# als244/ResNet

Measured on AMD Instinct MI355X. Metric: images/sec ResNet-50 fp32 224x224 batch256, higher is better.
Workload: dtype f32

## Files before the change

include/resnet_mi.h:

```cpp
#ifndef RESNET_MI_H
#define RESNET_MI_H
#include <stddef.h>
#include <stdint.h>

#ifdef __cplusplus
extern "C" {
#endif

typedef struct {
    char **labels;
    char **synsets;
    int *counts;
    int n_classes;
} Class_Metadata;

typedef struct {
    int input;
    int init_kernel_dim;
    int init_conv_filters;
    int init_conv_stride;
    int init_maxpool_dim;
    int init_maxpool_stride;
    int n_conv_blocks;
    int *is_block_spatial_reduction;
// ... 208 lines not shown
int mi_op_bn_fwd_add_relu(const float *x, const float *gamma, const float *beta, const float *residual, float *means,
                          float *vars, float *y, int N, int C, int H, float eps);
int mi_op_bn_bwd(const float *x, const float *gamma, const float *beta, const float *means, const float *vars,
                 const float *dy, const float *mask_src, float *dx, float *dgamma, float *dbeta, int N, int C, int H,
                 float eps, int mask_mode);
int mi_op_bn_bwd_gate(const float *x, const float *gamma, const float *beta, const float *means, const float *vars,
                      const float *dy, const float *mask_src, float *gated_out, float *dx, float *dgamma, float *dbeta, int N,
                      int C, int H, float eps);
int mi_op_maxpool_fwd(const float *x, float *y, int *max_inds, int N, int C, int H, int k, int stride);
int mi_op_maxpool_bwd(const int *max_inds, const float *dy, float *dx, int N, int C, int H, int k, int stride);
int mi_op_avgpool_fwd(const float *x, float *y, int N, int C, int H);
int mi_op_avgpool_bwd(const float *dy, float *dx, int N, int C, int H);
int mi_op_relu_deriv(const float *x, const float *up, float *out, size_t n);
int mi_op_matmul(const float *A, const float *B, float *out, int m, int k, int n);
int mi_op_matmul_lt(const float *A_kxm, const float *B, float *out, int m, int k, int n);
int mi_op_matmul_rt(const float *A, const float *B_nxk, float *out, int m, int k, int n);
int mi_op_softmax(const float *x, float *out, int N, int L);
int mi_op_ce_deriv(const float *pred, const int *labels, float *d, int N, int L);
int mi_op_adam(float *p, const float *g, float *m, float *v, size_t n, float lr, float wd, float b1, float b2,
               float cur_b1, float cur_b2, float eps, int *nan_flag_dev);
int mi_op_nhwc_to_nchw(const float *in, float *out, int N, int H, int W, int C);
int mi_debug_lds_fill(uint32_t word);
int mi_debug_poison_lds(void);
int mi_debug_lds_probe(uint32_t word, size_t out[4]);
int mi_debug_lds_geometry(size_t out[3]);
int mi_debug_lds_fill_mode(int on, uint32_t word);
size_t mi_debug_lds_fills(void);
int mi_debug_redzone(size_t zone_bytes, int fill_byte);
int mi_debug_redzone_check(void);
void mi_debug_redzone_stats(size_t *allocs_checked, size_t *zone_bytes_checked, size_t *live);
int mi_debug_trace_names(char *buf, size_t cap);
void mi_debug_trace_clear(void);
int mi_debug_conv_plan(int op, int N, int C, int H, int K, int k, int stride, int out[9]);
int mi_op_fill_uniform(float *out, size_t n, uint64_t seed, float lo, float hi);
enum { MI_ROUTE_DEFAULT = 0, MI_ROUTE_CL = 1, MI_ROUTE_CL2 = 2, MI_ROUTE_PW = 3 };
int mi_conv_plan(int dtype, int route, int op, int N, int C, int H, int K, int k, int stride, int out[7]);
enum { MI_FWD_F32, MI_FWD_BF16, MI_FWD_CL, MI_FWD_STEM_F32, MI_FWD_STEM_BF16, MI_FWD_PW  };
enum { MI_DG_F32, MI_DG_BF16, MI_DG_CL, MI_DG_CL2 };
enum { MI_WG_F32, MI_WG_BF16, MI_WG_CL, MI_WG_CL2, MI_WG_STEM_F32, MI_WG_STEM_BF16 };
int mi_layer_routes(int dtype, int policy, int N, int C, int H, int K, int k, int stride, int site, int out[4]);
enum {
    MI_K_NONE,
    MI_K_IGEMM,
    MI_K_GEMM1X1,
    MI_K_DCONV,
    MI_K_WGRADC,
    MI_K_WGRAD,
    MI_K_BGEMM,
    MI_K_PW_WGRAD,
    MI_K_CL_CONV,
    MI_K_CL_DGRAD2,
    MI_K_CL_WGRAD,
    MI_K_CL_WGRAD2,
    MI_K_ST32_FWD,
    MI_K_ST32_WGRAD,
    MI_K_ST_FWD,
    MI_K_ST_WGRAD
};
int mi_layer_kernels(int dtype, int policy, int N, int C, int H, int K, int k, int stride, int site, int out[3]);


enum { MI_DTYPE_F32 = 0, MI_DTYPE_BF16 = 1 };
int mi_trainer_set_dtype(Train_ResNet *t, int dtype);
int mi_trainer_get_dtype(const Train_ResNet *t);
enum { MI_STORE_FAST = 0, MI_STORE_RECOMPUTE_BN = 1, MI_STORE_FULL = 2 };
int mi_trainer_set_store_policy(Train_ResNet *t, int policy);
// ... 173 lines not shown
```

resnet_amd/binding.py:

```python
import ctypes as C
import os

_HERE = os.path.dirname(os.path.abspath(__file__))
LIB_PATH = os.environ.get("RESNET_MI_LIB") or os.path.join(_HERE, "libresnet_mi.so")

_fp = C.POINTER(C.c_float)
_ip = C.POINTER(C.c_int)


class Dims(C.Structure):
    _fields_ = [("input", C.c_int), ("init_kernel_dim", C.c_int), ("init_conv_filters", C.c_int),
                ("init_conv_stride", C.c_int), ("init_maxpool_dim", C.c_int), ("init_maxpool_stride", C.c_int),
                ("n_conv_blocks", C.c_int), ("is_block_spatial_reduction", _ip), ("final_depth", C.c_int),
                ("output", C.c_int)]


class BatchNorm(C.Structure):
    _fields_ = [("spatial_dim", C.c_int), ("depth", C.c_int), ("gamma", _fp), ("beta", _fp)]


class ConvBlock(C.Structure):
    _fields_ = [("incoming_filters", C.c_int), ("incoming_spatial_dim", C.c_int), ("reduced_depth", C.c_int),
                ("expanded_depth", C.c_int), ("stride", C.c_int), ("depth_reduction", _fp),
                ("norm_depth_reduction", C.POINTER(BatchNorm)), ("spatial", _fp), ("norm_spatial", C.POINTER(BatchNorm)),
# ... 191 lines not shown
    "mi_free": (None, [_vp]),
    "mi_op_conv_fwd": (_i, [_vp, _vp, _vp, _i, _i, _i, _i, _i, _i]),
    "mi_op_conv_dgrad": (_i, [_vp, _vp, _vp, _i, _i, _i, _i, _i, _i, _i]),
    "mi_op_conv_wgrad": (_i, [_vp, _vp, _vp, _i, _i, _i, _i, _i, _i]),
    "mi_op_bn_fwd": (_i, [_vp, _vp, _vp, _vp, _vp, _vp, _i, _i, _i, _f, _i]),
    "mi_op_bn_fwd_add_relu": (_i, [_vp, _vp, _vp, _vp, _vp, _vp, _vp, _i, _i, _i, _f]),
    "mi_op_bn_bwd": (_i, [_vp] * 10 + [_i, _i, _i, _f, _i]),
    "mi_op_bn_bwd_gate": (_i, [_vp] * 11 + [_i, _i, _i, _f]),
    "mi_op_maxpool_fwd": (_i, [_vp, _vp, _vp, _i, _i, _i, _i, _i]),
    "mi_op_maxpool_bwd": (_i, [_vp, _vp, _vp, _i, _i, _i, _i, _i]),
    "mi_op_avgpool_fwd": (_i, [_vp, _vp, _i, _i, _i]),
    "mi_op_avgpool_bwd": (_i, [_vp, _vp, _i, _i, _i]),
    "mi_op_relu_deriv": (_i, [_vp, _vp, _vp, _sz]),
    "mi_op_matmul": (_i, [_vp, _vp, _vp, _i, _i, _i]),
    "mi_op_matmul_lt": (_i, [_vp, _vp, _vp, _i, _i, _i]),
    "mi_op_matmul_rt": (_i, [_vp, _vp, _vp, _i, _i, _i]),
    "mi_op_softmax": (_i, [_vp, _vp, _i, _i]),
    "mi_op_ce_deriv": (_i, [_vp, _vp, _vp, _i, _i]),
    "mi_op_adam": (_i, [_vp, _vp, _vp, _vp, _sz, _f, _f, _f, _f, _f, _f, _f, _vp]),
    "mi_op_nhwc_to_nchw": (_i, [_vp, _vp, _i, _i, _i, _i]),
    "mi_op_fill_uniform": (_i, [_vp, _sz, _u64, _f, _f]),
    "mi_debug_poison_lds": (_i, []),
    "mi_debug_lds_fill": (_i, [C.c_uint32]),
    "mi_debug_lds_probe": (_i, [C.c_uint32, C.POINTER(_sz)]),
    "mi_debug_lds_geometry": (_i, [C.POINTER(_sz)]),
    "mi_debug_lds_fill_mode": (_i, [_i, C.c_uint32]),
    "mi_debug_lds_fills": (_sz, []),
    "mi_debug_redzone": (_i, [_sz, _i]),
    "mi_debug_redzone_check": (_i, []),
    "mi_debug_redzone_stats": (None, [C.POINTER(_sz)] * 3),
    "mi_debug_trace_names": (_i, [C.c_char_p, _sz]),
    "mi_debug_trace_clear": (None, []),
    "mi_debug_conv_plan": (_i, [_i] * 7 + [_vp]),
    "mi_conv_plan": (_i, [_i] * 9 + [_vp]),
    "mi_layer_routes": (_i, [_i] * 9 + [_vp]),
    "mi_layer_kernels": (_i, [_i] * 9 + [_vp]),
    "mi_debug_trainer_routes": (_i, [_T, _vp, _i]),
    "mi_trainer_set_dtype": (_i, [_T, _i]),
    "mi_trainer_get_dtype": (_i, [_T]),
    "mi_trainer_set_store_policy": (_i, [_T, _i]),
    "mi_trainer_activation_bytes": (_sz, [_T]),
    "mi_trainer_device_bytes": (_sz, [_T]),
    "mi_clear_error": (None, []),
    "mi_trainer_check_errors": (_i, [_T]),
    "mi_trainer_end_epoch": (None, [_T, _f, _f, _f]),
    "mi_trainer_set_optimizer": (_i, [_T, _i, _f, _f]),
    "mi_trainer_get_optimizer": (_i, [_T]),
    "mi_op_loss_head": (_i, [_vp, _vp, _vp, _vp, _vp, _vp, _i, _i, _f, _i, _vp, _vp]),
    "mi_trainer_set_loss": (_i, [_T, _f, _i, _i]),
    "mi_trainer_metrics": (_i, [_T, C.POINTER(MiLossMetrics), C.POINTER(MiLossMetrics), _i]),
    "mi_trainer_track_running_stats": (_i, [_T, _i, _f]),
    "mi_bn_unbias": (_f, [C.c_int64]),
    "mi_op_bn_running_update": (_i, [_vp, _vp, _vp, _vp, _i, _vp, _i, _f]),
    "mi_trainer_running_stats_channels": (_i, [_T]),
    "mi_trainer_get_running_stats": (_i, [_T, _vp, _vp]),
    "mi_trainer_set_running_stats": (_i, [_T, _vp, _vp]),
    "mi_trainer_running_updates": (C.c_int64, [_T]),
    "mi_trainer_eval_forward": (_i, [_T, _vp, _vp, _i, _i]),
    "mi_trainer_eval_metrics": (_i, [_T, C.POINTER(MiLossMetrics), C.POINTER(MiLossMetrics), _i]),
    "mi_trainer_eval_u8": (_i, [_T, _vp, _vp, C.c_int64, _i, _i, C.POINTER(MiLossMetrics)]),
    "mi_ema_weight": (_f, [C.c_double, _i, C.c_int64]),
    "mi_op_ema_update": (_i, [_vp, _vp, _sz, _f]),
    "mi_op_exchange": (_i, [_vp, _vp, _sz]),
    "mi_debug_ema_geometry": (None, [C.POINTER(_sz)]),
    "mi_trainer_set_ema": (_i, [_T, C.c_double, _i, _i]),
    "mi_trainer_ema_reset": (_i, [_T]),
# ... 108 lines not shown
```

resnet_amd/csrc/kernels_igemm.hip:

```cpp
#include "mi_common.hpp"
#include <type_traits>
#include "mi_device.h"

typedef float f32x16 __attribute__((ext_vector_type(16)));
typedef float pf4 __attribute__((ext_vector_type(4)));

enum { IG_FWD = 0, IG_DGRAD = 1, IG_WGRAD = 2 };

struct IgArgs {
    int N, C, K, H, W, Ho, Wo;
    int HW, P;
    int ncols;
    int mtiles;
    int tiles;
    int ctiles;
    int klen;
    FastDiv fdP, fdWo, fdM;
    int full, tsplit, tklen, cpt;
    FastDiv fdTs, fdCpt;
    float *tailbuf;
    float *bn_part;
    int bn_np;
    const float *bnb_x, *bnb_mask, *bnb_mean;
    float *bnb_part;
    int bnb_np;
};

__device__ __forceinline__ float ig_half_sum32(float v) {
    v += __int_as_float(__builtin_amdgcn_update_dpp(0, __float_as_int(v), 0xB1, 0xF, 0xF, true));
    v += __int_as_float(__builtin_amdgcn_update_dpp(0, __float_as_int(v), 0x4E, 0xF, 0xF, true));
    v += __int_as_float(__builtin_amdgcn_update_dpp(0, __float_as_int(v), 0x141, 0xF, 0xF, true));
    v += __int_as_float(__builtin_amdgcn_update_dpp(0, __float_as_int(v), 0x140, 0xF, 0xF, true));
    v += __int_as_float(__builtin_amdgcn_update_dpp(0, __float_as_int(v), 0x142, 0xA, 0xF, true));
    return v;
}

__device__ __forceinline__ void ig_half_stats(float x, int nv, int l31, float &mean, float &m2) {
    const float s = __shfl(x, (int)(threadIdx.x & 32), 64);
    const float d = l31 < nv ? x - s : 0.f;
    float sd = d, sq = d * d;
#pragma unroll
    for (int o = 16; o > 0; o >>= 1) { sd += __shfl_xor(sd, o, 64); sq += __shfl_xor(sq, o, 64); }
    const float inv = nv > 0 ? 1.0f / (float)nv : 0.f;
    mean = s + sd * inv;
    m2 = fmaxf(sq - sd * sd * inv, 0.f);
    if (nv <= 0) { mean = 0.f; m2 = 0.f; }
}
__device__ __forceinline__ void ig_merge(float &na, float &ma, float &qa, float nb, float mb, float qb) {
    const float n = na + nb;
    if (n > 0.f) {
        const float dlt = mb - ma, f = nb / n;
        ma = ma + dlt * f;
        qa = qa + qb + dlt * dlt * na * f;
    }
    na = n;
}

#define IG_BK 32
#ifdef IG_STAMP
__device__ unsigned long long ig_stamps[8 * 16384];
#define IG_T(slot) do { if (threadIdx.x == 0 && blockIdx.x < 16384 && blockIdx.y == 0) ig_stamps[blockIdx.x * 8 + (slot)] = __builtin_amdgcn_s_memtime(); } while (0)
#else
#define IG_T(slot) do { } while (0)
#endif
#ifndef IG_ABLATE
#define IG_ABLATE 0
#endif

template <int MODE, int KS, int S, int WMW, bool VBP = false>
__global__ void __launch_bounds__(256)
igemm_kernel(const float *__restrict__ Aop, const float *__restrict__ Bop, float *__restrict__ Out,
             const float *__restrict__ addend, const IgArgs g) {
    constexpr int BM = 64 * WMW;
    constexpr int TN = WMW == 2 ? 2 : 1;
    constexpr int WNC = 32 * TN;
    constexpr int T = KS * KS, PAD = KS / 2;
    constexpr int LDA = (MODE == IG_WGRAD) ? BM + 1 : BM + 4;
    constexpr int LDB = (MODE == IG_WGRAD) ? 129 : 132;
    constexpr int NA4 = BM / 32;
    constexpr int NAS = BM / 8;
    constexpr bool VB = VBP && KS == 1 && MODE != IG_WGRAD;
    constexpr bool CT64 = VBP && MODE == IG_WGRAD;
    extern __shared__ __attribute__((aligned(16))) float ig_smem[];
    float *As = ig_smem;
    float *Bs = ig_smem + 2 * IG_BK * LDA;
    const int tid = threadIdx.x, lane = tid & 63;
    const int wave = __builtin_amdgcn_readfirstlane(tid >> 6);
    const int wm = WMW == 2 ? wave >> 1 : 0, wn = WMW == 2 ? wave & 1 : wave;

    IG_T(0);
    uint32_t L = blockIdx.x;
    int tail_id = -1, it0 = 0, nt_slice = 0;
    uint32_t wg_split = blockIdx.y;
    if (MODE != IG_WGRAD && g.tsplit > 1 && L >= (uint32_t)g.full) {
        tail_id = (int)(L - (uint32_t)g.full);
        const uint32_t tl = fd_div((uint32_t)tail_id, g.fdTs);
        const int z = tail_id - (int)tl * g.tsplit;
        L = (uint32_t)g.full + tl;
        it0 = z * g.tklen;
        nt_slice = g.tklen;
    } else if (MODE == IG_WGRAD && gridDim.y >= 8) {
        const uint32_t T_ = gridDim.x, tot = T_ * gridDim.y, per = tot >> 3;
// ... 251 lines not shown
            __builtin_amdgcn_sched_barrier(0);
            if (grp < 8) { if (st) stash_part(buf ^ 1, grp); }
            else { if (ft) fetch_part(grp - 8); }
#pragma unroll
            for (int i = 0; i < 2; i++)
#pragma unroll
                for (int j = 0; j < TN; j++)
                    acc[i][j] = __builtin_amdgcn_mfma_f32_32x32x2f32(av[cur][i], bv[cur][j], acc[i][j], 0, 0, 0);
            __builtin_amdgcn_sched_barrier(0);
        }
        __syncthreads();
    };
    {
        constexpr std::true_type Y{};
        constexpr std::false_type NO{};
        int it = 0;
        for (; it + 2 < ntiles; it++) kstep(Y, Y, it & 1);
        if (it + 1 < ntiles) { kstep(Y, NO, it & 1); it++; }
        if (it < ntiles) kstep(NO, NO, it & 1);
    }

    IG_T(2);
    if (MODE != IG_WGRAD && tail_id >= 0) {
        float *tb = g.tailbuf + (size_t)tail_id * (BM * 128);
#pragma unroll
        for (int j = 0; j < TN; j++)
#pragma unroll
            for (int i = 0; i < 2; i++)
#pragma unroll
                for (int r = 0; r < 16; r++)
                    tb[(wm * 64 + i * 32 + (r & 3) + 8 * (r >> 2) + 4 * (lane >> 5)) * 128 + wn * WNC + j * 32 + (lane & 31)] = acc[i][j][r];
        return;
    }
    if (MODE == IG_DGRAD && S == 1 && g.bnb_part) {
        constexpr int PPT = 4 / WMW;
        if ((g.P & 3) == 0) {
            constexpr int CPR = WNC / 4, RPI = 64 / CPR, PITCH = WNC + 4;
            float *img = ig_smem + wave * (32 * PITCH);
            const int c4 = (lane % CPR) * 4, r0 = lane / CPR;
            const int col = n0 + wn * WNC + c4;
            const bool cok = col < g.ncols;
            const uint32_t jc = cok ? (uint32_t)col : 0u;
            const uint32_t nimg = fd_div(jc, g.fdP);
            const size_t coff = (size_t)nimg * g.C * g.HW + (jc - nimg * g.P);
            const size_t pplane = (size_t)g.bnb_np * g.C;
#pragma unroll
            for (int i = 0; i < 2; i++) {
#pragma unroll
                for (int j = 0; j < TN; j++)
#pragma unroll
                    for (int r = 0; r < 16; r++)
                        img[((r & 3) + 8 * (r >> 2) + 4 * (lane >> 5)) * PITCH + j * 32 + (lane & 31)] = acc[i][j][r];
#pragma unroll
                for (int ps = 0; ps < 32 / RPI; ps++) {
                    const int rl = ps * RPI + r0;
                    const int row = m0 + wm * 64 + i * 32 + rl;
                    const size_t o = coff + (size_t)row * g.HW;
                    const pf4 z = {0.f, 0.f, 0.f, 0.f};
                    pf4 v = *(const pf4 *)(img + rl * PITCH + c4);
                    pf4 xv = z, mv = z;
                    if (cok) {
                        if (addend) v += *(const pf4 *)(addend + o);
                        xv = *(const pf4 *)(g.bnb_x + o);
                        mv = *(const pf4 *)(g.bnb_mask + o);
                    }
                    const float mean = g.bnb_mean[row];
                    float s1 = 0.f, s2 = 0.f;
// ... 184 lines not shown
        for (int i = 0; i < 8; i++) {
            const size_t o = coff + (size_t)(m0 + row0 + i) * rstride;
            float r = v[i];
            if (MODE == IG_DGRAD && addend) r += addend[o];
            Out[o] = r;
        }
    }
    if (MODE == IG_FWD && g.bn_part) {
        constexpr int PPT = BM == 128 ? 2 : 4;
        const int lane = threadIdx.x & 63, l31 = lane & 31;
        const int c32 = (int)ct * 128 + (int)(threadIdx.x & 127 & ~31);
        const int nv = min(32, max(0, g.ncols - c32));
        const size_t plane = (size_t)g.bn_np * g.K;
#pragma unroll
        for (int i = 0; i < 8; i++) {
            float mj, qj, nj = (float)nv;
            ig_half_stats(v[i], nv, l31, mj, qj);
            int pp = (int)(threadIdx.x & 127) >> 5;
            if (PPT == 2) {
                const float n2 = __shfl_xor(nj, 32, 64), m2o = __shfl_xor(mj, 32, 64), q2 = __shfl_xor(qj, 32, 64);
                if (lane == 0) ig_merge(nj, mj, qj, n2, m2o, q2);
                pp >>= 1;
            }
            if (PPT == 2 ? lane == 0 : l31 == 0) {
                const size_t o = (size_t)(ct * PPT + pp) * g.K + m0 + row0 + i;
                g.bn_part[o] = nj;
                g.bn_part[plane + o] = mj;
                g.bn_part[2 * plane + o] = qj;
            }
        }
    }
}

template <int T>
__global__ void __launch_bounds__(256)
igemm_wt_kernel(const float *__restrict__ w, float *__restrict__ out, int K, int C, int to_tck) {
    __shared__ float tile[32][T * 32 + 1];
    const int k0 = blockIdx.y * 32, c0 = blockIdx.x * 32;
    for (int e = threadIdx.x; e < 32 * T * 32; e += 256) {
        const int kr = e / (T * 32), x = e - kr * (T * 32);
        tile[kr][x] = w[((size_t)(k0 + kr) * C + c0) * T + x];
    }
    __syncthreads();
    for (int e = threadIdx.x; e < T * 32 * 32; e += 256) {
        const int t = e >> 10, u = (e >> 5) & 31, v = e & 31;
        if (to_tck) out[((size_t)t * C + c0 + u) * K + k0 + v] = tile[v][u * T + t];
        else out[((size_t)t * K + k0 + u) * C + c0 + v] = tile[u][v * T + t];
    }
}

__global__ void __launch_bounds__(256)
igemm_wt_all_kernel(const mid_wt_entry *__restrict__ entries, const int *__restrict__ tile_entry) {
    __shared__ float tile[32][9 * 32 + 1];
    const mid_wt_entry E = entries[tile_entry[blockIdx.x]];
    const int tl = (int)blockIdx.x - E.tile0, ctiles = E.C / 32, T = E.T;
    const int c0 = (tl % ctiles) * 32, k0 = (tl / ctiles) * 32, row = T * 32;
    for (int e = threadIdx.x; e < 32 * row; e += 256) {
        const int kr = e / row, x = e - kr * row;
        tile[kr][x] = E.w[((size_t)(k0 + kr) * E.C + c0) * T + x];
    }
    __syncthreads();
    for (int e = threadIdx.x; e < T * 1024; e += 256) {
        const int t = e >> 10, u = (e >> 5) & 31, v = e & 31;
        if (E.fwd) E.fwd[((size_t)t * E.C + c0 + u) * E.K + k0 + v] = tile[v][u * T + t];
        if (E.dgrad) E.dgrad[((size_t)t * E.K + k0 + u) * E.C + c0 + v] = tile[u][v * T + t];
    }
// ... 195 lines not shown
    const int bm = (op == IGOP_FWD || stride == 1) ? igemm_pick_bm(M, mi_cdiv(g.ncols, 128), k * k * (red / IG_BK), k) : (M % 128 == 0 ? 128 : 64);
    g.mtiles = M / bm;
    g.tiles = g.mtiles * mi_cdiv(g.ncols, 128);
    g.fdM = make_fastdiv(g.mtiles);
    g.cpt = red / IG_BK; g.fdCpt = make_fastdiv(g.cpt);
    return bm;
}
static int igemm_plan_wgrad(IgArgs &g, int N, int C, int H, int K, int k, int stride, bool swapped, int *used) {
    int bm;
    if (swapped) {
        const int splits = igemm_wgrad_splits(N, K, H, C, 1, 1);
        igemm_geometry(g, N,  K, H,  C, 1);
        bm = C % 128 == 0 ? 128 : 64;
        g.mtiles = C / bm;
        g.ctiles = K / 128;
        g.tiles = g.mtiles * g.ctiles;
        g.klen = mi_cdiv(mi_cdiv(N * g.P, splits), IG_BK) * IG_BK;
    } else {
        const int T = k * k;
        const int splits = igemm_wgrad_splits(N, C, H, K, k, stride);
        igemm_geometry(g, N, C, H, K, stride);
        bm = K % 128 == 0 ? 128 : 64;
        g.mtiles = K / bm;
        g.ctiles = C / 128;
        g.tiles = C == 64 ? g.mtiles * ((T + 1) / 2) : g.mtiles * T * g.ctiles;
        g.klen = mi_cdiv(mi_cdiv(N * g.P, splits), IG_BK) * IG_BK;
    }
    g.fdM = make_fastdiv(g.mtiles);
    g.full = g.tiles; g.tsplit = 1; g.fdTs = make_fastdiv(1); g.cpt = 1; g.fdCpt = make_fastdiv(1);
    *used = mi_cdiv(N * g.P, g.klen);
    return bm;
}
static thread_local const char *ig_variant = "igemm_kernel";
template <int MODE, int KS, int S, int WMW, bool VB = false>
static int igemm_launch_t(hipStream_t st, dim3 grid, const float *A, const float *B, float *out, const float *addend, const IgArgs &g) {
    constexpr int BM = 64 * WMW;
    constexpr int LDA = (MODE == IG_WGRAD) ? BM + 1 : BM + 4, LDB = (MODE == IG_WGRAD) ? 129 : 132;
    constexpr size_t lds = (size_t)2 * IG_BK * (LDA + LDB) * sizeof(float);
    static int attr_set = 0;
    if (!attr_set) {
        if (lds > 64 * 1024 &&
            hipFuncSetAttribute((const void *)igemm_kernel<MODE, KS, S, WMW, VB>, hipFuncAttributeMaxDynamicSharedMemorySize, (int)lds) != hipSuccess) {
            mi_record_error("igemm_kernel", "cannot raise the dynamic LDS limit");
            return -1;
        }
        attr_set = 1;
    }
    hipLaunchKernelGGL((igemm_kernel<MODE, KS, S, WMW, VB>), grid, dim3(256), lds, st, A, B, out, addend, g);
    ig_variant = mi_trace_name("igemm_kernel<%s,k%d,s%d,bm%d%s%s>", MODE == IG_FWD ? "fwd" : MODE == IG_DGRAD ? "dgrad" : "wgrad", KS, S, BM, VB ? ",vb" : "",
                               g.tsplit > 1 ? ",tail" : "");
    return 0;
}
template <int MODE>
static int igemm_launch(hipStream_t st, dim3 grid, const float *A, const float *B, float *out, const float *addend, const IgArgs &g,
                        int k, int stride, int bm) {
#define IGL(KS_, S_)                                                                                      \
    if (k == KS_ && stride == S_)                                                                         \
        return bm == 128 ? igemm_launch_t<MODE, KS_, S_, 2>(st, grid, A, B, out, addend, g)               \
                         : igemm_launch_t<MODE, KS_, S_, 1>(st, grid, A, B, out, addend, g);
    if (MODE != IG_WGRAD && k == 1 && stride == 1 && g.P % 4 == 0)
        return bm == 128 ? igemm_launch_t<MODE, 1, 1, 2, true>(st, grid, A, B, out, addend, g)
                         : igemm_launch_t<MODE, 1, 1, 1, true>(st, grid, A, B, out, addend, g);
    if (MODE == IG_WGRAD && k == 3 && g.C == 64) {
        if (stride == 1) return bm == 128 ? igemm_launch_t<MODE, 3, 1, 2, true>(st, grid, A, B, out, addend, g) : igemm_launch_t<MODE, 3, 1, 1, true>(st, grid, A, B, out, addend, g);
        return bm == 128 ? igemm_launch_t<MODE, 3, 2, 2, true>(st, grid, A, B, out, addend, g) : igemm_launch_t<MODE, 3, 2, 1, true>(st, grid, A, B, out, addend, g);
    }
    IGL(1, 1) IGL(3, 1) IGL(3, 2)
#undef IGL
    return -2;
}
static int igemm_fam(int k) { return k == 1 ? MI_FAM_GEMM : MI_FAM_PCONV; }

extern "C" int mi_igemm_fwd(mid_stream s, mid_workspace *ws, const float *x, const float *w, float *y, int N, int C, int H, int K, int k,
                            int stride, mid_bn_parts *parts) {
    hipStream_t st = (hipStream_t)s;
    const int T = k * k;
    if (parts) parts->nparts = 0;
    if (!mi_igemm_supported(IGOP_FWD, N, C, H, K, k, stride)) { mi_record_error("mi_igemm_fwd", "shape not supported by the implicit GEMM"); return -2; }
    if (!ws || ws->wt_floats < (size_t)T * C * K) { mi_record_error("mi_igemm_fwd", "workspace too small"); return -3; }
    const float *A = ws->pre_fwd;
    if (!A) {
        if (k == 1) hipLaunchKernelGGL(igemm_wt_kernel<1>, dim3(C / 32, K / 32), dim3(256), 0, st, w, ws->wt, K, C, 1);
        else hipLaunchKernelGGL(igemm_wt_kernel<9>, dim3(C / 32, K / 32), dim3(256), 0, st, w, ws->wt, K, C, 1);
        MI_LAUNCH_CHECK("igemm_wt_kernel");
        A = ws->wt;
    }
    IgArgs g = {};
    const int bm = igemm_plan_tiles(g, IGOP_FWD, N, C, H, K, k, stride);
    igemm_tail_plan(g, T * g.cpt, ws->wt_floats >= (size_t)T * C * K + IG_TAIL_FLOATS ? ws->wt + (size_t)T * C * K : nullptr, bm);
    if (parts) {
        parts->nparts = 0;
        const int np = mi_cdiv(g.ncols, 128) * (bm == 128 ? 2 : 4);
        if (parts->buf && parts->floats >= (size_t)3 * np * K) { g.bn_part = parts->buf; g.bn_np = np; parts->nparts = np; }
    }
    mi_prof_begin(st, igemm_fam(k), 2.0 * T * (double)g.ncols * C * K,
                  4.0 * ((double)N * C * g.HW + (double)T * C * K + (double)g.ncols * K));
    int rc = igemm_launch<IG_FWD>(st, dim3(g.full + (g.tiles - g.full) * g.tsplit), A, x, y, nullptr, g, k, stride, bm);
    if (!rc && g.tsplit > 1) {
        if (bm == 128) hipLaunchKernelGGL((igemm_tail_reduce_kernel<IG_FWD, 128>), dim3(g.tiles - g.full, 8), dim3(256), 0, st, y, nullptr, g);
        else hipLaunchKernelGGL((igemm_tail_reduce_kernel<IG_FWD, 64>), dim3(g.tiles - g.full, 4), dim3(256), 0, st, y, nullptr, g);
    }
    mi_prof_end(st);
    if (rc) return rc;
    MI_LAUNCH_CHECK(ig_variant);
    return 0;
}

extern "C" int mi_igemm_dgrad(mid_stream s, mid_workspace *ws, const float *w, const float *dy, float *dx, const float *addend, int N,
                              int C, int H, int K, int k, int stride, mid_bn_bwd_parts *fz) {
    hipStream_t st = (hipStream_t)s;
    if (fz) fz->nparts = 0;
    if (!mi_igemm_supported(IGOP_DGRAD, N, C, H, K, k, stride)) { mi_record_error("mi_igemm_dgrad", "shape not supported by the implicit GEMM"); return -2; }
    const int T = k * k;
    const float *A = w;
    if (k == 3) {
        if (!ws || ws->wt_floats < (size_t)T * C * K) { mi_record_error("mi_igemm_dgrad", "workspace too small"); return -3; }
        if (ws->pre_dgrad) A = ws->pre_dgrad;
        else {
            hipLaunchKernelGGL(igemm_wt_kernel<9>, dim3(C / 32, K / 32), dim3(256), 0, st, w, ws->wt, K, C, 0);
            MI_LAUNCH_CHECK("igemm_wt_kernel");
// ... 56 lines not shown
                  4.0 * ((double)N * C * g.HW + (double)kd * K + (double)T * C * K));
    const int rc = igemm_launch<IG_WGRAD>(st, dim3(g.tiles, used), dy, x, ws->part, nullptr, g, k, stride, bm);
    mi_prof_end(st);
    if (rc) return rc;
    MI_LAUNCH_CHECK(ig_variant);
    const long KC = (long)K * C;
    MI_LAUNCH_CHECK(igemm_wgrad_reduce_launch(st, ws->part, dw, KC, k, used));
    return 0;
}

int mi_igemm_wgrad_reduce(hipStream_t st, const float *part, float *dw, int K, int C, int k, int splits) {
    const long KC = (long)K * C;
    MI_LAUNCH_CHECK(igemm_wgrad_reduce_launch(st, part, dw, KC, k, splits));
    return 0;
}

#ifdef IG_STAMP
extern "C" int mi_debug_igemm_stamps(unsigned long long *dst, int nblocks) {
    return hipMemcpyFromSymbol(dst, HIP_SYMBOL(ig_stamps), sizeof(unsigned long long) * 8 * (size_t)nblocks) == hipSuccess ? 0 : -1;
}
#endif

extern "C" int mid_igemm_plan(int op, int N, int C, int H, int K, int k, int stride, int out[9]) {
    for (int i = 0; i < 9; i++) out[i] = 0;
    if (!mi_igemm_supported(op, N, C, H, K, k, stride)) return 0;
    out[0] = 1;
    IgArgs g = {};
    if (op == IGOP_WGRAD) {
        int used;
        out[1] = igemm_plan_wgrad(g, N, C, H, K, k, stride, igemm_wgrad_swapped(C, K, k), &used);
        out[2] = g.tiles; out[3] = g.tiles; out[4] = 1; out[5] = g.klen / IG_BK; out[6] = used; out[7] = g.tiles; out[8] = mi_cdiv(N * g.P, IG_BK);
        return 1;
    }
    const int bm = igemm_plan_tiles(g, op, N, C, H, K, k, stride);
    float dummy;
    igemm_tail_plan(g, k * k * g.cpt, (op == IGOP_FWD || stride == 1) ? &dummy : nullptr, bm);
    out[1] = bm; out[2] = g.tiles; out[3] = g.full; out[4] = g.tsplit; out[5] = g.tklen; out[6] = 1;
    out[7] = g.full + (g.tiles - g.full) * g.tsplit; out[8] = k * k * g.cpt;
    return 1;
}
extern "C" int mid_wgrad_reduce_grouped(int K, int C, int splits) { return igemm_wgrad_reduce_grouped((long)K * C, splits) ? 1 : 0; }
extern "C" int mid_igemm_conv_plan(int op, int N, int C, int H, int K, int k, int stride, int out[7]) {
    int o[9];
    if (!mid_igemm_plan(op, N, C, H, K, k, stride, o)) return 0;
    out[0] = o[1]; out[1] = 128; out[2] = o[2]; out[3] = o[3]; out[4] = o[4]; out[5] = o[6];
    out[6] = op == IGOP_WGRAD && !igemm_wgrad_swapped(C, K, k) ? mid_wgrad_reduce_grouped(K, C, o[6]) : 0;
    return 1;
}

extern "C" int mid_conv_prelayout_all(mid_stream s, const mid_wt_entry *entries_dev, const int *tile_entry_dev, int ntiles) {
    if (ntiles <= 0) return 0;
    hipLaunchKernelGGL(igemm_wt_all_kernel, dim3(ntiles), dim3(256), 0, (hipStream_t)s, entries_dev, tile_entry_dev);
    MI_LAUNCH_CHECK("igemm_wt_all_kernel");
    return 0;
}
```

resnet_amd/csrc/mi_device.h:

```cpp
#ifndef MI_DEVICE_H
#define MI_DEVICE_H
#include <stddef.h>
#include <stdint.h>
#ifdef __cplusplus
extern "C" {
#endif

typedef void *mid_stream;
typedef void *mid_event;

enum { MID_F32 = 0, MID_BF16 = 1 };

int mid_device_count(void);
int mid_set_device(int dev);
const char *mid_last_error(void);
void mid_clear_error(void);
void *mid_malloc(size_t bytes);
void mid_free(void *p);
int mid_redzone(size_t zone_bytes, int fill_byte);
int mid_redzone_check(void);
void mid_redzone_stats(size_t *allocs_checked, size_t *zone_bytes_checked, size_t *live);
int mid_trace_names(char *buf, size_t cap);
void mid_trace_clear(void);
void *mid_malloc_host(size_t bytes);
// ... 92 lines not shown
int mid_cl_relayout(mid_stream s, const void *x, void *xp, int N, int C, int H, int parity);
int mid_cl_fwd(mid_stream s, const void *xp, const void *a_tiles, void *y, int N, int C, int H, int K, int stride, mid_bn_parts *parts);
int mid_cl_dgrad(mid_stream s, const void *dyp, const void *a_tiles, void *dx, const void *addend, int N, int C, int H, int K);
int mid_cl_wgrad_supported(int N, int C, int H, int K, int stride);
size_t mid_cl_wgrad_part_floats(int N, int C, int H, int K, int stride);
int mid_cl_pw_supported(int N, int C, int H, int K);
int mid_cl_relayout_dense(mid_stream s, const void *x, void *xp, int N, int C, int H);
int mid_cl_pw_fwd(mid_stream s, const void *xc, const void *a_tiles, void *y, int N, int C, int H, int K, mid_bn_parts *parts);
int mid_cl_wgrad2_supported(int N, int C, int H, int K, int stride);
size_t mid_cl_wgrad2_part_floats(int N, int C, int H, int K, int stride);
int mid_cl_wgrad2(mid_stream s, const void *xp, const void *dyp, float *dw, float *part, size_t part_floats, int N, int C, int H, int K, int stride);
int mid_pw_wgrad_supported(int N, int C, int H, int K);
size_t mid_pw_wgrad_part_floats(int N, int C, int H, int K);
int mid_pw_wgrad(mid_stream s, const void *x, const void *dy, float *dw, float *part, size_t part_floats, int N, int C, int H, int K);
int mid_cl_wgrad(mid_stream s, const void *xp, const void *dy, float *dw, float *part, size_t part_floats, int N, int C, int H, int K, int stride);
int mid_cl_dgrad2_supported(int N, int C, int H, int K);
size_t mid_cl_dgrad2_operand_bytes(int N, int K, int Ho);
int mid_cl_relayout_end(mid_stream s, const void *dy, void *dyp, int N, int K, int Ho);
int mid_cl_dgrad2(mid_stream s, const void *dyp, const void *a_tiles, void *dx, int N, int C, int H, int K);
size_t mid_stem_f32_xp_bytes(int N, int H);
int mid_stem_fwd_f32(mid_stream s, const float *x, const float *w, float *y, void *xp, size_t xp_bytes, float *scratch, size_t scratch_floats,
                     int N, int H, mid_bn_parts *parts);
int mid_stem_wgrad_f32(mid_stream s, const void *xp, const float *dy, float *dw, float *scratch, size_t scratch_floats, int N, int H);
int mid_stem_bf16_supported(int C, int H, int K, int k, int stride);
size_t mid_stem_bf16_xp_bytes(int N, int H);
size_t mid_stem_bf16_part_floats(int N, int H);
int mid_stem_fwd_bf16(mid_stream s, const float *x, const float *w, void *y, int y_dt, void *xp, size_t xp_bytes, float *scratch, size_t scratch_floats,
                      int N, int H, mid_bn_parts *parts);
int mid_stem_wgrad_bf16(mid_stream s, const void *xp, const void *dy, int dy_dt, float *dw, float *scratch, size_t scratch_floats, int N, int H);
int mid_f32_to_bf16(mid_stream s, const float *in, void *out, size_t n);
int mid_bf16_to_f32(mid_stream s, const void *in, float *out, size_t n);

int mid_igemm_plan(int op, int N, int C, int H, int K, int k, int stride, int out[9]);
int mid_igemm_conv_plan(int op, int N, int C, int H, int K, int k, int stride, int out[7]);
int mid_bf16_conv_plan(int op, int N, int C, int H, int K, int k, int stride, int out[7]);
int mid_cl_conv_plan(int route, int op, int N, int C, int H, int K, int k, int stride, int out[7]);
int mid_wgrad_reduce_grouped(int K, int C, int splits);

int mid_gemm_nn(mid_stream s, const float *A, const float *B, float *out, int m, int k, int n);
int mid_gemm_tn(mid_stream s, const float *At, const float *B, float *out, int m, int k, int n);
int mid_gemm_nt(mid_stream s, const float *A, const float *Bt, float *out, int m, int k, int n);

size_t mid_bn_ws_floats(int C);
int mid_bn_fwd(mid_stream s, float *stats_ws, const float *x, const float *gamma, const float *beta,
               const float *residual, float *means, float *vars, float *y, float *xhat_out, float *norm_out, int N,
               int C, int P, float eps, int relu);
int mid_bn_fwd_parts(mid_stream s, float *stats_ws, const mid_bn_parts *parts, const float *x, const float *gamma,
                     const float *beta, const float *residual, float *means, float *vars, float *y, float *xhat_out,
                     float *norm_out, int N, int C, int P, float eps, int relu);
int mid_bn_bwd(mid_stream s, float *stats_ws, const float *x, const float *gamma, const float *beta,
               const float *means, const float *vars, const float *dy, const float *mask_src, float *dx,
               float *dgamma, float *dbeta, int N, int C, int P, float eps, int mask_mode);

int mid_bn_bwd_gate(mid_stream s, float *stats_ws, const float *x, const float *gamma, const float *beta,
                    const float *means, const float *vars, const float *dy, const float *mask_src, float *gated_out,
                    float *dx, float *dgamma, float *dbeta, int N, int C, int P, float eps);

int mid_bn_fwd_t(mid_stream s, float *stats_ws, const mid_bn_parts *parts, const void *x, int x_dt, const float *gamma,
                 const float *beta, const void *residual, float *means, float *vars, void *y, int a_dt, float *xhat_out,
                 float *norm_out, int N, int C, int P, float eps, int relu, void *ycl, int Hcl);
void mid_bn_set_sync(void *comm, int world, float *tmp, size_t tmp_floats, int force);
int mid_bn_debug_merge(mid_stream s, int R, int C, float *means, float *vars, float *dgamma, float *dbeta, float *sums_out, float *tmp);
int mid_bn_stats_t(mid_stream s, float *stats_ws, const void *x, int x_dt, float *means, float *vars, int N, int C, int P);
int mid_bn_apply_t(mid_stream s, const void *x, int x_dt, const float *gamma, const float *beta, const void *residual,
                   const float *means, const float *vars, void *y, int a_dt, int N, int C, int P, float eps, int relu, void *ycl, int Hcl);
typedef struct { const float *means, *vars; int first, off, C; float unbias; } mid_bn_run_entry;
// ... 85 lines not shown
```

resnet_amd/csrc/ops.c:

```c
#include <math.h>
#include <stdint.h>
#include <stdlib.h>
#include <string.h>
#include "mi_host.h"

void *mi_malloc(size_t bytes) {
    char *p = (char *)mid_malloc(bytes + 2 * MI_GUARD);
    return p ? p + MI_GUARD : NULL;
}
void mi_free(void *p) { if (p) mid_free((char *)p - MI_GUARD); }

static int finish(int rc) {
    mid_stream_sync(mi_global()->compute);
    if (rc) return rc;
    return mid_last_error()[0] ? -1 : 0;
}

typedef struct { MiLayer L; MiLayerWs w; mid_wt_entry we; mid_stream s; int rc; } OpConv;
static MiOptions op_options(void) {
    MiOptions env, o = {.bnfuse_bwd = 1, .bnfuse_bwd_f32 = 7};
    mi_read_options(&env);
    o.igemm = env.igemm; o.pw_wgrad = env.pw_wgrad;
    return o;
}
// ... 274 lines not shown
    return finish(mid_erase_batch(mi_global()->compute, images_nchw, n, (size_t)image_size, dim, boxes_host, fill_host->mode, fill_host->value,
                                  fill_host->std, fill_host->noise_seed, first_row));
}
void mi_debug_erase_geometry(size_t out[4]) { mid_erase_geometry(out); }
_Static_assert(sizeof(MiTaRow) == sizeof(mid_ta_row), "MiTaRow and mid_ta_row are one layout");
size_t mi_ta_workspace_bytes(int n, int dim) { return mid_ta_workspace_bytes(n, dim); }
int mi_op_trivial_augment(float *images_nchw, int n, int image_size, int dim, const MiTaRow *rows_host, void *workspace_dev) {
    if (!rows_host || !workspace_dev) { mi_record_host_error("mi_op_trivial_augment", "rows_host / workspace_dev is NULL"); return -1; }
    if (image_size < 1) { mi_record_host_error("mi_op_trivial_augment", "image_size = 3 dim^2"); return -1; }
    return finish(mid_trivial_augment(mi_global()->compute, images_nchw, n, (size_t)image_size, dim, (const mid_ta_row *)rows_host, workspace_dev));
}
void mi_debug_ta_geometry(size_t out[4]) { mid_ta_geometry(out); }
int mi_op_fill_uniform(float *out, size_t n, uint64_t seed, float lo, float hi) { return finish(mid_fill_uniform(mi_global()->compute, out, n, seed, 0, lo, hi)); }
int mi_debug_lds_fill(uint32_t word) { return finish(mid_debug_lds_fill(word)); }
int mi_debug_poison_lds(void) { return mi_debug_lds_fill(0xFFFFFFFFu); }
int mi_debug_lds_probe(uint32_t word, size_t out[4]) { return finish(mid_debug_lds_probe(word, out)); }
int mi_debug_lds_geometry(size_t out[3]) { return finish(mid_debug_lds_geometry(out)); }
int mi_debug_lds_fill_mode(int on, uint32_t word) { return finish(mid_debug_lds_fill_mode(on, word)); }
size_t mi_debug_lds_fills(void) { return mid_debug_lds_fills(); }
int mi_debug_redzone(size_t zone_bytes, int fill_byte) { return mid_redzone(zone_bytes, fill_byte); }
int mi_debug_redzone_check(void) { return mid_redzone_check(); }
void mi_debug_redzone_stats(size_t *allocs_checked, size_t *zone_bytes_checked, size_t *live) { mid_redzone_stats(allocs_checked, zone_bytes_checked, live); }
int mi_debug_trace_names(char *buf, size_t cap) { return mid_trace_names(buf, cap); }
void mi_debug_trace_clear(void) { mid_trace_clear(); }
static int on_igemm(int op, int N, int C, int H, int K, int k, int stride) {
    const MiOptions opt = op_options();
    return op >= 0 && op <= 2 && mi_layer_f32_kernel(&opt, op, N, C, H, K, k, stride) == MI_K_IGEMM;
}
int mi_debug_conv_plan(int op, int N, int C, int H, int K, int k, int stride, int out[9]) {
    if (on_igemm(op, N, C, H, K, k, stride)) return mid_igemm_plan(op, N, C, H, K, k, stride, out);
    for (int i = 0; i < 9; i++) out[i] = 0;
    return 0;
}
int mi_conv_plan(int dtype, int route, int op, int N, int C, int H, int K, int k, int stride, int out[7]) {
    for (int i = 0; i < 7; i++) out[i] = 0;
    int ok = 0;
    if (op < 0 || op > 2) ok = 0;
    else if (dtype == MI_DTYPE_F32 && route == MI_ROUTE_DEFAULT) ok = on_igemm(op, N, C, H, K, k, stride) && mid_igemm_conv_plan(op, N, C, H, K, k, stride, out);
    else if (dtype == MI_DTYPE_BF16 && route == MI_ROUTE_DEFAULT) ok = mid_bf16_conv_plan(op, N, C, H, K, k, stride, out);
    else if (dtype == MI_DTYPE_BF16 && route >= MI_ROUTE_CL && route <= MI_ROUTE_PW) ok = mid_cl_conv_plan(route, op, N, C, H, K, k, stride, out);
    if (!ok) { for (int i = 0; i < 7; i++) out[i] = 0; return -2; }
    return 0;
}

int mi_op_convert(const void *in, int in_dt, void *out, int out_dt, size_t n) {
    if (in_dt == MID_F32 && out_dt == MID_BF16) return finish(mid_f32_to_bf16(mi_global()->compute, (const float *)in, out, n));
    if (in_dt == MID_BF16 && out_dt == MID_F32) return finish(mid_bf16_to_f32(mi_global()->compute, in, (float *)out, n));
    return -2;
}
int mi_op_conv_fwd_bf16(const void *x, const float *w, void *y, int N, int C, int H, int K, int k, int stride) {
    return op_conv(MID_BF16, MI_FWD_BF16, OFF, OFF, x, w, NULL, y, NULL, N, C, H, K, k, stride);
}
int mi_op_conv_dgrad_bf16(const float *w, const void *dy, void *dx, int N, int C, int H, int K, int k, int stride, int to_add) {
    return op_conv(MID_BF16, OFF, MI_DG_BF16, OFF, NULL, w, dy, dx, to_add ? dx : NULL, N, C, H, K, k, stride);
}
int mi_op_conv_wgrad_bf16(const void *x, const void *dy, float *dw, int N, int C, int H, int K, int k, int stride) {
    return op_conv(MID_BF16, OFF, OFF, MI_WG_BF16, x, NULL, dy, dw, NULL, N, C, H, K, k, stride);
}
static int op_dgrad_bn_bwd(int dt, const float *w, const void *dy, const void *addend, void *gated, int N, int C, int H, int K, int k, int stride,
                           const void *bn_x, const void *mask, const float *gamma, const float *beta, const float *means, const float *vars,
                           float eps, void *bn_dx, float *dgamma, float *dbeta) {
    OpConv o;
    const size_t bytes = (size_t)N * C * H * H * (dt == MID_BF16 ? 2 : 4);
    mid_bn_bwd_parts fz = {NULL}, req;
    void *tmp = NULL;
    const MiOptions opt = op_options();
// ... 144 lines not shown
```

Baseline: 2440.

## Add dedicated pointwise forward kernel reusing activation tile across output-channel tiles

New measurement: 2449, median of 6. About the same (+0.4%).

```diff
diff --git a/include/resnet_mi.h b/include/resnet_mi.h
--- a/include/resnet_mi.h
+++ b/include/resnet_mi.h
@@ -264,6 +264,8 @@
 int mi_debug_trace_names(char *buf, size_t cap);
 void mi_debug_trace_clear(void);
 int mi_debug_conv_plan(int op, int N, int C, int H, int K, int k, int stride, int out[9]);
+int mi_debug_igemm_pw(int mode);
+int mi_debug_pw_plan(int op, int N, int C, int H, int K, int k, int stride, int out[8]);
 int mi_op_fill_uniform(float *out, size_t n, uint64_t seed, float lo, float hi);
 enum { MI_ROUTE_DEFAULT = 0, MI_ROUTE_CL = 1, MI_ROUTE_CL2 = 2, MI_ROUTE_PW = 3 };
 int mi_conv_plan(int dtype, int route, int op, int N, int C, int H, int K, int k, int stride, int out[7]);
diff --git a/resnet_amd/binding.py b/resnet_amd/binding.py
--- a/resnet_amd/binding.py
+++ b/resnet_amd/binding.py
@@ -247,6 +247,8 @@
     "mi_debug_trace_names": (_i, [C.c_char_p, _sz]),
     "mi_debug_trace_clear": (None, []),
     "mi_debug_conv_plan": (_i, [_i] * 7 + [_vp]),
+    "mi_debug_igemm_pw": (_i, [_i]),
+    "mi_debug_pw_plan": (_i, [_i] * 7 + [_vp]),
     "mi_conv_plan": (_i, [_i] * 9 + [_vp]),
     "mi_layer_routes": (_i, [_i] * 9 + [_vp]),
     "mi_layer_kernels": (_i, [_i] * 9 + [_vp]),
diff --git a/resnet_amd/csrc/kernels_igemm.hip b/resnet_amd/csrc/kernels_igemm.hip
--- a/resnet_amd/csrc/kernels_igemm.hip
+++ b/resnet_amd/csrc/kernels_igemm.hip
@@ -24,6 +24,7 @@
     const float *bnb_x, *bnb_mask, *bnb_mean;
     float *bnb_part;
     int bnb_np;
+    int pw_g, pw_groups;
 };
 
 __device__ __forceinline__ float ig_half_sum32(float v) {
@@ -67,7 +68,7 @@
 #define IG_ABLATE 0
 #endif
 
-template <int MODE, int KS, int S, int WMW, bool VBP = false>
+template <int MODE, int KS, int S, int WMW, bool VBP = false, bool FZ = false>
 __global__ void __launch_bounds__(256)
 igemm_kernel(const float *__restrict__ Aop, const float *__restrict__ Bop, float *__restrict__ Out,
              const float *__restrict__ addend, const IgArgs g) {
@@ -385,7 +386,7 @@
                     tb[(wm * 64 + i * 32 + (r & 3) + 8 * (r >> 2) + 4 * (lane >> 5)) * 128 + wn * WNC + j * 32 + (lane & 31)] = acc[i][j][r];
         return;
     }
-    if (MODE == IG_DGRAD && S == 1 && g.bnb_part) {
+    if (MODE == IG_DGRAD && S == 1 && FZ) {
         constexpr int PPT = 4 / WMW;
         if ((g.P & 3) == 0) {
             constexpr int CPR = WNC / 4, RPI = 64 / CPR, PITCH = WNC + 4;
@@ -636,6 +637,123 @@
     }
 }
 
+#define PW_LDB 132
+#define PW_LDA 68
+#define PW_PITCH 36
+template <int NK>
+__global__ void __launch_bounds__(256)
+igemm_pw_kernel(const float *__restrict__ Aop, const float *__restrict__ Bop, float *__restrict__ Out, const IgArgs g) {
+    constexpr int RED = 32 * NK;
+    constexpr int NB4 = RED / 8;
+    constexpr int NA4 = RED / 16;
+    extern __shared__ __attribute__((aligned(16))) float ig_smem[];
+    float *Bs = ig_smem;
+    float *As = ig_smem + RED * PW_LDB;
+    const int tid = threadIdx.x, lane = tid & 63;
+    const int wave = __builtin_amdgcn_readfirstlane(tid >> 6);
+    uint32_t L = blockIdx.x;
+    {
+        const uint32_t per = (uint32_t)g.tiles >> 3;
+        if (L < per * 8) L = (L & 7) * per + (L >> 3);
+    }
+    const uint32_t ct = fd_div(L, g.fdM);
+    const int mt0 = (int)(L - ct * (uint32_t)g.pw_groups) * g.pw_g, mt1 = min(g.mtiles, mt0 + g.pw_g);
+    const int n0 = (int)ct * 128;
+    const pf4 z4 = {0.f, 0.f, 0.f, 0.f};
+
+    {
+        const int j = n0 + (tid & 31) * 4;
+        const bool jin = j < g.ncols;
+        const uint32_t jc = jin ? (uint32_t)j : (uint32_t)g.ncols - 4u;
+        const uint32_t n = fd_div(jc, g.fdP);
+        const uint32_t p = jc - n * g.P;
+        const char *xb = (const char *)Bop + (size_t)(n * (uint32_t)(g.C * g.HW) + p + (uint32_t)(tid >> 5) * g.HW) * 4;
+        pf4 rb[NB4];
+#pragma unroll
+        for (int q = 0; q < NB4; q++) rb[q] = *(const pf4 *)(xb + (size_t)(8 * q) * g.HW * 4);
+#pragma unroll
+        for (int q = 0; q < NB4; q++) *(pf4 *)(Bs + ((tid >> 5) + 8 * q) * PW_LDB + (tid & 31) * 4) = jin ? rb[q] : z4;
+    }
+    const int a_i = (tid & 15) * 4, a_k = tid >> 4;
+    pf4 ra[NA4];
+    auto fetch_a = [&](const int mt) {
+        const float *ap = Aop + (size_t)a_k * g.K + mt * 64 + a_i;
+#pragma unroll
+        for (int q = 0; q < NA4; q++) ra[q] = *(const pf4 *)(ap + (size_t)(16 * q) * g.K);
+    };
+    auto stash_a = [&]() {
+#pragma unroll
+        for (int q = 0; q < NA4; q++) *(pf4 *)(As + (a_k + 16 * q) * PW_LDA + a_i) = ra[q];
+    };
+    fetch_a(mt0);
+    stash_a();
+    __syncthreads();
+
+    const int fr = lane & 31, fk = lane >> 5;
+    const float *as = As + fk * PW_LDA + fr;
+    const float *bs = Bs + fk * PW_LDB + wave * 32 + fr;
+    float *img = As + wave * (32 * PW_PITCH);
+    const int c4 = (lane & 7) * 4, r0 = lane >> 3;
+    const int col = n0 + wave * 32 + c4;
+    const bool cok = col < g.ncols;
+    const uint32_t jcs = cok ? (uint32_t)col : 0u;
+    const uint32_t nimg = fd_div(jcs, g.fdP);
+    const size_t coff = (size_t)nimg * g.K * g.P + (jcs - nimg * g.P);
+    const int nv = min(32, max(0, g.ncols - (n0 + wave * 32)));
+    const size_t plane = (size_t)g.bn_np * g.K;
+
+    for (int mt = mt0; mt < mt1; mt++) {
+        f32x16 acc[2];
+#pragma unroll
+        for (int i = 0; i < 2; i++)
+#pragma unroll
+            for (int r = 0; r < 16; r++) acc[i][r] = 0.f;
+#pragma unroll
+        for (int k2 = 0; k2 < RED; k2 += 2) {
+            const float a0 = as[k2 * PW_LDA], a1 = as[k2 * PW_LDA + 32], b = bs[k2 * PW_LDB];
+            acc[0] = __builtin_amdgcn_mfma_f32_32x32x2f32(a0, b, acc[0], 0, 0, 0);
+            acc[1] = __builtin_amdgcn_mfma_f32_32x32x2f32(a1, b, acc[1], 0, 0, 0);
+        }
+        __syncthreads();
+        if (mt + 1 < mt1) fetch_a(mt + 1);
+        const int m0 = mt * 64;
+#pragma unroll
+        for (int i = 0; i < 2; i++) {
+#pragma unroll
+            for (int r = 0; r < 16; r++) img[((r & 3) + 8 * (r >> 2) + 4 * (lane >> 5)) * PW_PITCH + (lane & 31)] = acc[i][r];
+#pragma unroll
+            for (int ps = 0; ps < 4; ps++) {
+                const int rl = ps * 8 + r0;
+                const pf4 v = *(const pf4 *)(img + rl * PW_PITCH + c4);
+                if (cok) *(pf4 *)(Out + coff + (size_t)(m0 + i * 32 + rl) * g.P) = v;
+            }
+            if (g.bn_part && lane < 32) {
+                const float *rw = img + lane * PW_PITCH;
+                const float s0 = rw[0];
+                float sd = 0.f, sq = 0.f;
+#pragma unroll 8
+                for (int c = 0; c < 32; c++) {
+                    const float x = rw[c];
+                    const float d = c < nv ? x - s0 : 0.f;
+                    sd += d;
+                    sq = fmaf(d, d, sq);
+                }
+                const float inv = nv > 0 ? 1.0f / (float)nv : 0.f;
+                const size_t o = (size_t)(ct * 4 + wave) * g.K + m0 + i * 32 + lane;
+                g.bn_part[o] = (float)nv;
+                g.bn_part[plane + o] = nv > 0 ? s0 + sd * inv : 0.f;
+                const float m2 = sq - sd * sd * inv;
+                g.bn_part[2 * plane + o] = fmaxf(m2, 0.f);
+            }
+        }
+        if (mt + 1 < mt1) {
+            __syncthreads();
+            stash_a();
+            __syncthreads();
+        }
+    }
+}
+
 template <int T>
 __global__ void __launch_bounds__(256)
 igemm_wt_kernel(const float *__restrict__ w, float *__restrict__ out, int K, int C, int to_tck) {
@@ -897,7 +1015,7 @@
     return bm;
 }
 static thread_local const char *ig_variant = "igemm_kernel";
-template <int MODE, int KS, int S, int WMW, bool VB = false>
+template <int MODE, int KS, int S, int WMW, bool VB = false, bool FZ = false>
 static int igemm_launch_t(hipStream_t st, dim3 grid, const float *A, const float *B, float *out, const float *addend, const IgArgs &g) {
     constexpr int BM = 64 * WMW;
     constexpr int LDA = (MODE == IG_WGRAD) ? BM + 1 : BM + 4, LDB = (MODE == IG_WGRAD) ? 129 : 132;
@@ -905,13 +1023,13 @@
     static int attr_set = 0;
     if (!attr_set) {
         if (lds > 64 * 1024 &&
-            hipFuncSetAttribute((const void *)igemm_kernel<MODE, KS, S, WMW, VB>, hipFuncAttributeMaxDynamicSharedMemorySize, (int)lds) != hipSuccess) {
+            hipFuncSetAttribute((const void *)igemm_kernel<MODE, KS, S, WMW, VB, FZ>, hipFuncAttributeMaxDynamicSharedMemorySize, (int)lds) != hipSuccess) {
             mi_record_error("igemm_kernel", "cannot raise the dynamic LDS limit");
             return -1;
         }
         attr_set = 1;
     }
-    hipLaunchKernelGGL((igemm_kernel<MODE, KS, S, WMW, VB>), grid, dim3(256), lds, st, A, B, out, addend, g);
+    hipLaunchKernelGGL((igemm_kernel<MODE, KS, S, WMW, VB, FZ>), grid, dim3(256), lds, st, A, B, out, addend, g);
     ig_variant = mi_trace_name("igemm_kernel<%s,k%d,s%d,bm%d%s%s>", MODE == IG_FWD ? "fwd" : MODE == IG_DGRAD ? "dgrad" : "wgrad", KS, S, BM, VB ? ",vb" : "",
                                g.tsplit > 1 ? ",tail" : "");
     return 0;
@@ -919,6 +1037,18 @@
 template <int MODE>
 static int igemm_launch(hipStream_t st, dim3 grid, const float *A, const float *B, float *out, const float *addend, const IgArgs &g,
                         int k, int stride, int bm) {
+    if constexpr (MODE == IG_DGRAD) {
+        if (stride == 1 && g.bnb_part) {
+            const bool vb = k == 1 && g.P % 4 == 0;
+#define IGZ(KS_, VB_)                                                                                     \
+    if (k == KS_ && vb == VB_)                                                                            \
+        return bm == 128 ? igemm_launch_t<IG_DGRAD, KS_, 1, 2, VB_, true>(st, grid, A, B, out, addend, g) \
+                         : igemm_launch_t<IG_DGRAD, KS_, 1, 1, VB_, true>(st, grid, A, B, out, addend, g);
+            IGZ(1, true) IGZ(1, false) IGZ(3, false)
+#undef IGZ
+            return -2;
+        }
+    }
 #define IGL(KS_, S_)                                                                                      \
     if (k == KS_ && stride == S_)                                                                         \
         return bm == 128 ? igemm_launch_t<MODE, KS_, S_, 2>(st, grid, A, B, out, addend, g)               \
@@ -935,6 +1065,61 @@
     return -2;
 }
 static int igemm_fam(int k) { return k == 1 ? MI_FAM_GEMM : MI_FAM_PCONV; }
+
+#define PW_MIN_COLTILES 512
+#define PW_GROUP 4
+static int ig_pw_mode = -1;
+extern "C" int mid_debug_igemm_pw(int mode) {
+    if (mode < -1 || mode > 1) return -1;
+    ig_pw_mode = mode;
+    return 0;
+}
+static size_t igemm_pw_lds(int C) {
+    const size_t a = (size_t)C * PW_LDA, img = (size_t)4 * 32 * PW_PITCH;
+    return ((size_t)C * PW_LDB + (a > img ? a : img)) * sizeof(float);
+}
+static bool igemm_pw_takes(int op, int N, int C, int H, int K, int k, int stride) {
+    if (ig_pw_mode == 0 || op != IGOP_FWD || k != 1 || stride != 1 || (H * H) % 4 != 0) return false;
+    if (!mi_igemm_supported(op, N, C, H, K, k, stride)) return false;
+    if (C != 64 || K < 2 * C) return false;
+    if (ig_pw_mode == 1) return true;
+    return mi_cdiv((long)N * H * H, 128) >= PW_MIN_COLTILES && (double)N * K * H * H < 536870912.0;
+}
+static void igemm_pw_plan(IgArgs &g, int N, int C, int H, int K) {
+    igemm_geometry(g, N, C, H, K, 1);
+    g.mtiles = K / 64;
+    g.pw_g = PW_GROUP;
+    g.pw_groups = mi_cdiv(g.mtiles, g.pw_g);
+    g.tiles = g.pw_groups * mi_cdiv(g.ncols, 128);
+    g.fdM = make_fastdiv(g.pw_groups);
+    g.cpt = C / IG_BK; g.fdCpt = make_fastdiv(g.cpt);
+    g.full = g.tiles; g.tsplit = 1; g.tklen = g.cpt; g.fdTs = make_fastdiv(1);
+}
+extern "C" int mid_igemm_pw_plan(int op, int N, int C, int H, int K, int k, int stride, int out[8]) {
+    for (int i = 0; i < 8; i++) out[i] = 0;
+    if (!igemm_pw_takes(op, N, C, H, K, k, stride)) return 0;
+    IgArgs g = {};
+    igemm_pw_plan(g, N, C, H, K);
+    out[0] = 1; out[1] = 64; out[2] = g.pw_g; out[3] = g.pw_groups; out[4] = mi_cdiv(g.ncols, 128); out[5] = g.mtiles; out[6] = g.tiles;
+    out[7] = (int)igemm_pw_lds(C);
+    return 1;
+}
+template <int NK>
+static int igemm_pw_launch_t(hipStream_t st, const float *A, const float *x, float *y, const IgArgs &g) {
+    const size_t lds = igemm_pw_lds(32 * NK);
+    static int attr_set = 0;
+    if (!attr_set) {
+        if (lds > 64 * 1024 &&
+            hipFuncSetAttribute((const void *)igemm_pw_kernel<NK>, hipFuncAttributeMaxDynamicSharedMemorySize, (int)lds) != hipSuccess) {
+            mi_record_error("igemm_pw_kernel", "cannot raise the dynamic LDS limit");
+            return -1;
+        }
+        attr_set = 1;
+    }
+    hipLaunchKernelGGL((igemm_pw_kernel<NK>), dim3(g.tiles), dim3(256), lds, st, A, x, y, g);
+    ig_variant = mi_trace_name("igemm_pw_kernel<fwd,bm64,nk%d,g%d>", NK, g.pw_g);
+    return 0;
+}
 
 extern "C" int mi_igemm_fwd(mid_stream s, mid_workspace *ws, const float *x, const float *w, float *y, int N, int C, int H, int K, int k,
                             int stride, mid_bn_parts *parts) {
@@ -951,6 +1136,19 @@
         A = ws->wt;
     }
     IgArgs g = {};
+    if (igemm_pw_takes(IGOP_FWD, N, C, H, K, k, stride)) {
+        igemm_pw_plan(g, N, C, H, K);
+        if (parts) {
+            const int np = mi_cdiv(g.ncols, 128) * 4;
+            if (parts->buf && parts->floats >= (size_t)3 * np * K) { g.bn_part = parts->buf; g.bn_np = np; parts->nparts = np; }
+        }
+        mi_prof_begin(st, igemm_fam(k), 2.0 * (double)g.ncols * C * K, 4.0 * ((double)N * C * g.HW + (double)C * K + (double)g.ncols * K));
+        const int rc = igemm_pw_launch_t<2>(st, A, x, y, g);
+        mi_prof_end(st);
+        if (rc) return rc;
+        MI_LAUNCH_CHECK(ig_variant);
+        return 0;
+    }
     const int bm = igemm_plan_tiles(g, IGOP_FWD, N, C, H, K, k, stride);
     igemm_tail_plan(g, T * g.cpt, ws->wt_floats >= (size_t)T * C * K + IG_TAIL_FLOATS ? ws->wt + (size_t)T * C * K : nullptr, bm);
     if (parts) {
@@ -1073,6 +1271,11 @@
         out[2] = g.tiles; out[3] = g.tiles; out[4] = 1; out[5] = g.klen / IG_BK; out[6] = used; out[7] = g.tiles; out[8] = mi_cdiv(N * g.P, IG_BK);
         return 1;
     }
+    if (igemm_pw_takes(op, N, C, H, K, k, stride)) {
+        igemm_pw_plan(g, N, C, H, K);
+        out[1] = 64; out[2] = g.tiles; out[3] = g.tiles; out[4] = 1; out[5] = g.cpt; out[6] = 1; out[7] = g.tiles; out[8] = g.cpt;
+        return 1;
+    }
     const int bm = igemm_plan_tiles(g, op, N, C, H, K, k, stride);
     float dummy;
     igemm_tail_plan(g, k * k * g.cpt, (op == IGOP_FWD || stride == 1) ? &dummy : nullptr, bm);
diff --git a/resnet_amd/csrc/mi_device.h b/resnet_amd/csrc/mi_device.h
--- a/resnet_amd/csrc/mi_device.h
+++ b/resnet_amd/csrc/mi_device.h
@@ -148,6 +148,8 @@
 int mid_bf16_to_f32(mid_stream s, const void *in, float *out, size_t n);
 
 int mid_igemm_plan(int op, int N, int C, int H, int K, int k, int stride, int out[9]);
+int mid_igemm_pw_plan(int op, int N, int C, int H, int K, int k, int stride, int out[8]);
+int mid_debug_igemm_pw(int mode);
 int mid_igemm_conv_plan(int op, int N, int C, int H, int K, int k, int stride, int out[7]);
 int mid_bf16_conv_plan(int op, int N, int C, int H, int K, int k, int stride, int out[7]);
 int mid_cl_conv_plan(int route, int op, int N, int C, int H, int K, int k, int stride, int out[7]);
diff --git a/resnet_amd/csrc/ops.c b/resnet_amd/csrc/ops.c
--- a/resnet_amd/csrc/ops.c
+++ b/resnet_amd/csrc/ops.c
@@ -330,6 +330,12 @@
     for (int i = 0; i < 9; i++) out[i] = 0;
     return 0;
 }
+int mi_debug_igemm_pw(int mode) { return mid_debug_igemm_pw(mode); }
+int mi_debug_pw_plan(int op, int N, int C, int H, int K, int k, int stride, int out[8]) {
+    if (on_igemm(op, N, C, H, K, k, stride)) return mid_igemm_pw_plan(op, N, C, H, K, k, stride, out);
+    for (int i = 0; i < 8; i++) out[i] = 0;
+    return 0;
+}
 int mi_conv_plan(int dtype, int route, int op, int N, int C, int H, int K, int k, int stride, int out[7]) {
     for (int i = 0; i < 7; i++) out[i] = 0;
     int ok = 0;
```
